# slitvinov/PINN_for_quantum_wavefunction_surfaces

Measured on NVIDIA B200. Metric: collocation points/sec per training step (fwd+lap+bwd), higher is better.
Workload: dtype f32

## Files before the change

pinn_for_quantum_wavefunction_surfaces_b200/csrc/pinn_device.cuh:

```cuda
#pragma once
#include "pinn_common.cuh"
#include "pinn_launch.h"

namespace pinn {

constexpr int ROWH = 64;
constexpr int ROWE = 32;
constexpr int EVAL_STASH = 2 * 32 * ROWH;
constexpr int ENET_STASH = 2 * 32 * ROWE;

__host__ __device__ constexpr int swz_tc(int row) { return ((((row & 3) << 1) | ((row >> 2) & 1)) << 2); }

__device__ __forceinline__ float rcp_approx(float x) {
  float r;
  asm("rcp.approx.ftz.f32 %0, %1;" : "=f"(r) : "f"(x));
  return r;
}
constexpr float NEG_LOG2E = -1.4426950408889634f;
__device__ __forceinline__ float ex2_approx(float x) {
  float e;
  asm("ex2.approx.ftz.f32 %0, %1;" : "=f"(e) : "f"(x));
  return e;
}

// ... 31 lines not shown
__device__ __forceinline__ float2 f2bc(float x) { return make_float2(x, x); }
__device__ __forceinline__ float2 f2neg(float2 a) { return make_float2(-a.x, -a.y); }
__device__ __forceinline__ float2 f2mul(float2 a, float2 b) { return __fmul2_rn(a, b); }
__device__ __forceinline__ float2 f2add(float2 a, float2 b) { return __fadd2_rn(a, b); }
__device__ __forceinline__ float2 f2fma(float2 a, float2 b, float2 c) { return __ffma2_rn(a, b, c); }

template <int ROW>
__device__ __forceinline__ float2 colsum2(const float* __restrict__ base, int col2, int half) {
  const float* b = base + half * 16 * ROW;
  float2 s0 = make_float2(0.0f, 0.0f), s1 = make_float2(0.0f, 0.0f);
#pragma unroll
  for (int p = 0; p < 16; p += 2) {
    s0 = __fadd2_rn(s0, *reinterpret_cast<const float2*>(b + p * ROW + (col2 ^ swz_tc(p))));
    s1 = __fadd2_rn(s1, *reinterpret_cast<const float2*>(b + (p + 1) * ROW + (col2 ^ swz_tc(p + 1))));
  }
  return __fadd2_rn(s0, s1);
}
template <int ROW>
__device__ __forceinline__ void colsum2_w(const float* __restrict__ base, int col2, int half, float wgt, float2& plain,
                                          float2& weighted) {
  const float* b = base + half * 16 * ROW;
  float2 s0 = make_float2(0.0f, 0.0f), s1 = s0, t0 = s0, t1 = s0;
  const int r0 = half * 16;
#pragma unroll
  for (int p = 0; p < 16; p += 2) {
    const float2 v0 = *reinterpret_cast<const float2*>(b + p * ROW + (col2 ^ swz_tc(p)));
    const float2 v1 = *reinterpret_cast<const float2*>(b + (p + 1) * ROW + (col2 ^ swz_tc(p + 1)));
    const float w0 = __shfl_sync(0xffffffffu, wgt, r0 + p), w1 = __shfl_sync(0xffffffffu, wgt, r0 + p + 1);
    s0 = __fadd2_rn(s0, v0); s1 = __fadd2_rn(s1, v1);
    t0 = __ffma2_rn(v0, make_float2(w0, w0), t0);
    t1 = __ffma2_rn(v1, make_float2(w1, w1), t1);
  }
  plain = __fadd2_rn(s0, s1);
  weighted = __fadd2_rn(t0, t1);
}

struct Geom {
  float f1, f2, ir1, ir2, al1, al2, al11, al12, al22;
  float R;
};

struct RawPt {
  float dx1, dx2, y, z, R;
};
__device__ __forceinline__ RawPt load_raw(const StepParams& p, long long i) {
  RawPt r;
  if (p.in_f64) {
    const double xd = ((const double*)p.x)[i], Rd = ((const double*)p.R)[i];
    r.dx1 = (float)(xd - Rd);
    r.dx2 = (float)(xd + Rd);
    r.y = (float)((const double*)p.y)[i];
    r.z = (float)((const double*)p.z)[i];
    r.R = (float)Rd;
  } else {
    const float xf = ((const float*)p.x)[i];
    r.R = ((const float*)p.R)[i];
    r.dx1 = xf - r.R;
    r.dx2 = xf + r.R;
    r.y = ((const float*)p.y)[i];
    r.z = ((const float*)p.z)[i];
  }
  return r;
}
__device__ __forceinline__ Geom geom_from_raw(const RawPt& r) {
  Geom g;
  const float yz = fmaf(r.y, r.y, r.z * r.z);
  const float q1 = fmaf(r.dx1, r.dx1, yz), q2 = fmaf(r.dx2, r.dx2, yz);
  g.ir1 = rsqrtf(q1);
  g.ir2 = rsqrtf(q2);
  const float r1 = q1 * g.ir1, r2 = q2 * g.ir2;
  g.f1 = __expf(-r1);
  g.f2 = __expf(-r2);
  const float c12 = fmaf(r.dx1, r.dx2, yz) * g.ir1 * g.ir2;
  g.al1 = g.f1 * fmaf(-2.0f, g.ir1, 1.0f);
  g.al2 = g.f2 * fmaf(-2.0f, g.ir2, 1.0f);
  g.al11 = g.f1 * g.f1;
  g.al22 = g.f2 * g.f2;
  g.al12 = 2.0f * g.f1 * g.f2 * c12;
  g.R = r.R;
  return g;
}
__device__ __forceinline__ Geom load_geom(const StepParams& p, long long i) { return geom_from_raw(load_raw(p, i)); }

__device__ __forceinline__ void build_weight_image(const float* __restrict__ th, Wts* __restrict__ out, int t, int nt) {
  for (int i = t; i < NH; i += nt) {
    const float a = th[O_W1 + 2 * i], b = th[O_W1 + 2 * i + 1];
    out->w0[i] = a; out->w1[i] = b; out->b1[i] = th[O_B1 + i];
    out->ww00[i] = a * a; out->ww01[i] = a * b; out->ww11[i] = b * b;
    out->b2[i] = th[O_B2 + i]; out->wo[i] = th[O_WO + i];
    out->w0s[i] = a * NEG_LOG2E; out->w1s[i] = b * NEG_LOG2E;
    out->b1s[i] = th[O_B1 + i] * NEG_LOG2E; out->b2s[i] = th[O_B2 + i] * NEG_LOG2E;
  }
  for (int i = t; i < NE; i += nt) {
    out->WE1[i] = th[O_WE1 + i]; out->bE1[i] = th[O_BE1 + i];
    out->bE2[i] = th[O_BE2 + i]; out->wE[i] = th[O_WE + i];
    out->WE1s[i] = th[O_WE1 + i] * NEG_LOG2E; out->bE1s[i] = th[O_BE1 + i] * NEG_LOG2E;
    out->bE2s[i] = th[O_BE2 + i] * NEG_LOG2E;
  }
  for (int i = t; i < 12; i += nt) {
    const bool in = i < NL;
    out->WgL[i] = in ? th[O_WGL + i] : 0.0f;
    out->bgL[i] = in ? th[O_BGL + i] : 0.0f;
    out->wg[i] = in ? th[O_WG + i] : 0.0f;
    out->WgLs[i] = in ? th[O_WGL + i] * NEG_LOG2E : 0.0f;
    out->bgLs[i] = in ? th[O_BGL + i] * NEG_LOG2E : 0.0f;
  }
  if (t == 0) { out->bo = th[O_BO]; out->bE = th[O_BE]; out->bg = th[O_BG]; out->pad0 = 0.0f; }
  auto put = [](float* hi, float* lo, int off, float v) {
    uint32_t h, l;
    split_tf32_rn(v, h, l);
    hi[off] = __uint_as_float(h);
    lo[off] = __uint_as_float(l);
  };
  for (int i = t; i < NH * NH; i += nt) {
    const int j = i / NH, k = i % NH;
    const float wjk = th[O_W2 + i];
    const float a = th[O_W1 + 2 * k], b = th[O_W1 + 2 * k + 1];
    put(out->BS[0], out->BS[1], umma_off(j, k, NH), wjk);
    put(out->BSP[0], out->BSP[1], umma_off(j, k, 2 * NH), wjk * a);
    put(out->BSP[0], out->BSP[1], umma_off(NH + j, k, 2 * NH), wjk * b);
    put(out->BSPP[0], out->BSPP[1], umma_off(j, k, 3 * NH), wjk * (a * a));
    put(out->BSPP[0], out->BSPP[1], umma_off(NH + j, k, 3 * NH), wjk * (a * b));
    put(out->BSPP[0], out->BSPP[1], umma_off(2 * NH + j, k, 3 * NH), wjk * (b * b));
    put(out->BWT[0], out->BWT[1], umma_off(k, j, NH), wjk);
  }
  for (int i = t; i < NE * NE; i += nt) {
    const int j = i / NE, k = i % NE;
    put(out->BE[0], out->BE[1], umma_off(j, k, NE), th[O_WE2 + i]);
    put(out->BET[0], out->BET[1], umma_off(k, j, NE), th[O_WE2 + i]);
  }
}

__device__ __forceinline__ void st_relaxed_sys_v2(unsigned int* p, unsigned int a, unsigned int b) {
  asm volatile("st.relaxed.sys.global.v2.u32 [%0], {%1, %2};" ::"l"(p), "r"(a), "r"(b) : "memory");
}
__device__ __forceinline__ uint2 ld_relaxed_sys_v2(const unsigned int* p) {
  uint2 v;
  asm volatile("ld.relaxed.sys.global.v2.u32 {%0, %1}, [%2];" : "=r"(v.x), "=r"(v.y) : "l"(p) : "memory");
  return v;
}
__device__ __forceinline__ double ld_acquire_gpu(const double* p) {
  double v;
  asm volatile("ld.acquire.gpu.global.f64 %0, [%1];" : "=d"(v) : "l"(p) : "memory");
  return v;
}
__device__ __forceinline__ void st_release_sys(unsigned long long* p, unsigned long long v) {
  asm volatile("st.release.sys.global.u64 [%0], %1;" ::"l"(p), "l"(v) : "memory");
}
__device__ __forceinline__ unsigned long long ld_acquire_sys(const unsigned long long* p) {
  unsigned long long v;
  asm volatile("ld.acquire.sys.global.u64 %0, [%1];" : "=l"(v) : "l"(p) : "memory");
  return v;
}

__device__ __forceinline__ float2 sigm2_pre(const float2 up) {
  const float2 d = __fadd2_rn(make_float2(ex2_approx(up.x), ex2_approx(up.y)), make_float2(1.0f, 1.0f));
  return make_float2(rcp_approx(d.x), rcp_approx(d.y));
}

__device__ __forceinline__ float2 one_minus_sigm2(const float2 e, const float2 s) {
  return make_float2(__saturatef(__fmul_rn(e.x, s.x)), __saturatef(__fmul_rn(e.y, s.y)));
}

__device__ __forceinline__ float2 sigm2_pre(const float2 up, float2& om) {
  const float2 e = make_float2(ex2_approx(up.x), ex2_approx(up.y));
  const float2 d = __fadd2_rn(e, make_float2(1.0f, 1.0f));
  const float2 s = make_float2(rcp_approx(d.x), rcp_approx(d.y));
  om = one_minus_sigm2(e, s);
  return s;
}

__device__ __forceinline__ float2 one_minus_sigm2_pre(const float2 up, const float2 s) {
  return one_minus_sigm2(make_float2(ex2_approx(up.x), ex2_approx(up.y)), s);
}

__device__ __forceinline__ float2 quad_form2(float al11, float al12, float al22, float2 v1, float2 v2) {
  return f2fma(f2mul(f2bc(al11), v1), v1, f2fma(f2mul(f2bc(al12), v1), v2, f2mul(f2mul(f2bc(al22), v2), v2)));
}

#define LD4(ptr) (*reinterpret_cast<const float4*>(ptr))
#define ST4(ptr, a, b, c, d) (*reinterpret_cast<float4*>(ptr) = make_float4(a, b, c, d))

}
```

pinn_for_quantum_wavefunction_surfaces_b200/csrc/pinn_step_tc.cu:

```cuda
#include <cstring>
#include <type_traits>

#include "pinn_tc.cuh"

#ifdef PINN_TIMELINE
__device__ long long g_timeline[16 * 32];
#define TL(i) do { if (blockIdx.x == 0 && c.tl_it == 3 && (threadIdx.x & 31) == 0) g_timeline[(threadIdx.x >> 5) * 32 + (i)] = clock64(); } while (0)
extern "C" int pinn_debug_timeline(long long* out) { return (int)cudaMemcpyFromSymbol(out, g_timeline, sizeof(g_timeline)); }
__device__ long long g_timeline_k[48];
__device__ long long g_timeline_cta[2 * 256];
extern "C" int pinn_debug_timeline_cta(long long* out) { return (int)cudaMemcpyFromSymbol(out, g_timeline_cta, sizeof(g_timeline_cta)); }
#define TLK(i) do { if (blockIdx.x == 0 && threadIdx.x == 0) g_timeline_k[(i)] = clock64(); \
                    if (threadIdx.x == 0 && ((i) == 0 || (i) == 41)) { unsigned long long t_; asm volatile("mov.u64 %0, %%globaltimer;" : "=l"(t_)); \
                      g_timeline_cta[blockIdx.x * 2 + ((i) == 41)] = (long long)t_; } } while (0)
extern "C" int pinn_debug_timeline_kernel(long long* out) { return (int)cudaMemcpyFromSymbol(out, g_timeline_k, sizeof(g_timeline_k)); }
#else
#define TL(i) do { } while (0)
#define TLK(i) do { } while (0)
#endif

namespace pinn {


template <int NEV>
__host__ __device__ constexpr int tc_group_stash_floats() { return NEV * EVAL_STASH + ENET_STASH; }
constexpr int GEO_BYTES = 2 * 128 * 12 * 4;
template <int NEV>
__host__ __device__ constexpr size_t tc_smem_bytes() {
  return sizeof(Wts) + 64  + sizeof(float2) * 4 * 2 * 3 * 32 + sizeof(float) * 4 * tc_group_stash_floats<NEV>() +
         COORD_STAGES * COORD_STAGE_BYTES + GEO_BYTES;
}

__device__ __forceinline__ void cp_async4(uint32_t dst, const void* src) {
  asm volatile("cp.async.ca.shared.global [%0], [%1], 4;" ::"r"(dst), "l"(src) : "memory");
}
__device__ __forceinline__ void cp_async8(uint32_t dst, const void* src) {
  asm volatile("cp.async.ca.shared.global [%0], [%1], 8;" ::"r"(dst), "l"(src) : "memory");
}
__device__ __forceinline__ void cp_async_commit() { asm volatile("cp.async.commit_group;" ::: "memory"); }
__device__ __forceinline__ void cp_async_wait_all() { asm volatile("cp.async.wait_group 0;" ::: "memory"); }

__device__ __forceinline__ void coord_stage_issue(const StepParams& p, unsigned char* buf, int slot, long long i) {
  const uint32_t b = smem_u32(buf);
  if (p.in_f64) {
    cp_async8(b + 0 * COORD_COL_BYTES + slot * 8, (const double*)p.x + i);
    cp_async8(b + 1 * COORD_COL_BYTES + slot * 8, (const double*)p.y + i);
    cp_async8(b + 2 * COORD_COL_BYTES + slot * 8, (const double*)p.z + i);
    cp_async8(b + 3 * COORD_COL_BYTES + slot * 8, (const double*)p.R + i);
  } else {
    cp_async4(b + 0 * COORD_COL_BYTES + slot * 4, (const float*)p.x + i);
    cp_async4(b + 1 * COORD_COL_BYTES + slot * 4, (const float*)p.y + i);
    cp_async4(b + 2 * COORD_COL_BYTES + slot * 4, (const float*)p.z + i);
    cp_async4(b + 3 * COORD_COL_BYTES + slot * 4, (const float*)p.R + i);
  }
  if (p.mask) cp_async4(b + 4 * COORD_COL_BYTES + slot * 4, (const void*)((uintptr_t)(p.mask + i) & ~(uintptr_t)3));
}
__device__ __forceinline__ void coord_stage_issue_bulk(const StepParams& p, unsigned char* buf, uint64_t* bar, long long st) {
  const uint32_t b = smem_u32(buf), mb = smem_u32(bar);
  const uint32_t colb = p.in_f64 ? 1024u : 512u;
  const uint32_t total = 4u * colb + (p.mask ? 128u : 0u);
  asm volatile("fence.proxy.async.shared::cta;" ::: "memory");
  asm volatile("mbarrier.arrive.expect_tx.shared::cta.b64 _, [%0], %1;" ::"r"(mb), "r"(total) : "memory");
  const char* src[4] = {(const char*)p.x, (const char*)p.y, (const char*)p.z, (const char*)p.R};
#pragma unroll
  for (int c = 0; c < 4; c++)
    asm volatile("cp.async.bulk.shared::cluster.global.mbarrier::complete_tx::bytes [%0], [%1], %2, [%3];" ::"r"(b + c * COORD_COL_BYTES),
                 "l"(src[c] + (size_t)st * colb), "r"(colb), "r"(mb)
                 : "memory");
  if (p.mask)
    asm volatile("cp.async.bulk.shared::cluster.global.mbarrier::complete_tx::bytes [%0], [%1], %2, [%3];" ::"r"(b + 4 * COORD_COL_BYTES),
                 "l"(p.mask + (size_t)st * 128), "r"(128u), "r"(mb)
                 : "memory");
}
__device__ __forceinline__ RawPt coord_stage_read(const StepParams& p, const unsigned char* buf, int slot) {
  RawPt r;
  if (p.in_f64) {
    const double xd = *(const double*)(buf + 0 * COORD_COL_BYTES + slot * 8), Rd = *(const double*)(buf + 3 * COORD_COL_BYTES + slot * 8);
    r.dx1 = (float)(xd - Rd);
    r.dx2 = (float)(xd + Rd);
    r.y = (float)*(const double*)(buf + 1 * COORD_COL_BYTES + slot * 8);
    r.z = (float)*(const double*)(buf + 2 * COORD_COL_BYTES + slot * 8);
    r.R = (float)Rd;
  } else {
    const float xf = *(const float*)(buf + 0 * COORD_COL_BYTES + slot * 4);
    r.R = *(const float*)(buf + 3 * COORD_COL_BYTES + slot * 4);
    r.dx1 = xf - r.R;
    r.dx2 = xf + r.R;
    r.y = *(const float*)(buf + 1 * COORD_COL_BYTES + slot * 4);
    r.z = *(const float*)(buf + 2 * COORD_COL_BYTES + slot * 4);
  }
  return r;
}

__device__ __forceinline__ void tc_role_sync(const TcCtx& c) {
  tc_wait_st();
  tc_fence_before();
  if (c.issuer) named_barrier(c.bar_id, 128);
  else asm volatile("bar.arrive %0, %1;" ::"r"(c.bar_id), "r"(128) : "memory");
}

template <bool STASH>
// ... 506 lines not shown
      ch[20 + i] = gs.x; ch[20 + i + 1] = gs.y;
    }
    ch[30] = gate_grads ? gbar : 0.0f;
    ch[31] = Ebar;
#pragma unroll
    for (int c4 = 0; c4 < 32; c4 += 4) ST4(&E1row[c4 ^ sx], ch[c4], ch[c4 + 1], ch[c4 + 2], ch[c4 + 3]);
  }
  __syncwarp();
  {
    float2 plain, weighted;
    colsum2_w<ROWE>(Vs, 2 * (lane & 15), lane >> 4, R, plain, weighted);
    acc2(acc.s2, weighted);
    acc2(acc.s3, plain);
  }
  acc2(acc.s4, colsum2<ROWE>(E1s, 2 * (lane & 15), lane >> 4));
  __syncwarp();
}

template <typename EntryOf>
__device__ __forceinline__ void fold_pair(float* __restrict__ myrow, float2 v, int lane, EntryOf entry_of) {
  v.x += __shfl_xor_sync(0xffffffffu, v.x, 16);
  v.y += __shfl_xor_sync(0xffffffffu, v.y, 16);
  if (lane < 16) {
    const int a = entry_of(2 * lane), b = entry_of(2 * lane + 1);
    if (a >= 0) myrow[a] = v.x;
    if (b >= 0) myrow[b] = v.y;
  }
}

constexpr int TC_REG_MLP = 184, TC_REG_ENET = 136;
static_assert(128 * TC_REG_ENET + 256 * TC_REG_MLP <= 384 * 168, "register rebalancing must fit the launch allocation");

struct TcParamsPlain {
  StepParams p;
  double w[4];
};
struct TcParamsInline {
  StepParams p;
  double w[4];
  alignas(16) float theta[NTHETA + 3];
};

template <int NEV, bool TRAIN, bool INLINE>
__global__ void __launch_bounds__((NEV + 1) * 128, 1)
pinn_step_tc_kernel(const __grid_constant__ typename std::conditional<INLINE, TcParamsInline, TcParamsPlain>::type q) {
  const StepParams& p = q.p;
  constexpr int G = 4;
  extern __shared__ __align__(128) unsigned char smem_raw[];
  Wts& w = *reinterpret_cast<Wts*>(smem_raw);
  uint64_t* mbars = reinterpret_cast<uint64_t*>(smem_raw + sizeof(Wts));
  uint32_t* tmem_slot = reinterpret_cast<uint32_t*>(smem_raw + sizeof(Wts) + 32);
  uint64_t* cfull = reinterpret_cast<uint64_t*>(smem_raw + sizeof(Wts) + 40);
  float2* mbox = reinterpret_cast<float2*>(smem_raw + sizeof(Wts) + 64);
  float* stash = reinterpret_cast<float*>(smem_raw + sizeof(Wts) + 64 + sizeof(float2) * G * 2 * 3 * 32);
  unsigned char* cstage = smem_raw + tc_smem_bytes<NEV>() - COORD_STAGES * COORD_STAGE_BYTES - GEO_BYTES;
  float4* geo = reinterpret_cast<float4*>(smem_raw + tc_smem_bytes<NEV>() - GEO_BYTES);

  const int tid = threadIdx.x, lane = tid & 31;
  const int warp = __shfl_sync(0xffffffffu, tid >> 5, 0);
  const int role = warp >> 2, grp = warp & 3;
  const bool is_mlp = role < NEV;
  const int sx = swz_tc(lane);
  TLK(0);
  uint32_t* clk0_slot = reinterpret_cast<uint32_t*>(smem_raw + sizeof(Wts) + 36);
  unsigned long long* ns0_slot = reinterpret_cast<unsigned long long*>(smem_raw + sizeof(Wts) + 56);
  if (blockIdx.x == 0 && tid == 0) {
    unsigned long long ns0;
    asm volatile("mov.u64 %0, %%globaltimer;" : "=l"(ns0));
    *ns0_slot = ns0;
    *clk0_slot = (uint32_t)clock();
  }

  if (warp == 0) {
    asm volatile("tcgen05.alloc.cta_group::1.sync.aligned.shared::cta.b32 [%0], 512;" ::"r"(smem_u32(tmem_slot)) : "memory");
    asm volatile("tcgen05.relinquish_alloc_permit.cta_group::1.sync.aligned;" ::: "memory");
  }
  if (tid == 32) {
#pragma unroll
    for (int i = 0; i < 4; i++) asm volatile("mbarrier.init.shared::cta.b64 [%0], 1;" ::"r"(smem_u32(&mbars[i])));
#pragma unroll
    for (int i = 0; i < COORD_STAGES; i++) asm volatile("mbarrier.init.shared::cta.b64 [%0], 1;" ::"r"(smem_u32(&cfull[i])));
    asm volatile("fence.mbarrier_init.release.cluster;" ::: "memory");
  }
  tc_fence_before();
  __syncthreads();
  tc_fence_after();
  pdl_wait();
  const int slot = grp * 32 + lane;
  const bool stager = !is_mlp && !p.grid.on;
  const bool cbulk = INLINE && TRAIN && !p.grid.on &&
                     ((((uintptr_t)p.x | (uintptr_t)p.y | (uintptr_t)p.z | (uintptr_t)p.R | (uintptr_t)p.mask) & 15u) == 0);
  auto tile_bulk = [&](long long st) { return INLINE && cbulk && (st * 128 + 128 <= p.n); };
  const bool bulk_issuer = stager && grp == 0 && lane == 0;
  if (stager && tile_bulk(blockIdx.x)) {
    if (bulk_issuer) coord_stage_issue_bulk(p, cstage, &cfull[0], blockIdx.x);
  } else if (stager) {
    const long long i0 = (long long)blockIdx.x * 128 + slot;
    coord_stage_issue(p, cstage, slot, i0 < p.n ? i0 : p.n - 1);
    cp_async_commit();
  }

  {
    float* th_s = stash;
    constexpr uint32_t TH_BULK = (NTHETA * 4 / 16) * 16;
    const bool bulk_ok = ((uintptr_t)p.theta & 15u) == 0;
    if constexpr (INLINE) {
      const float4* src = reinterpret_cast<const float4*>(q.theta);
      for (int j = warp; j < (NTHETA + 3) / 4; j += (NEV + 1) * 4) {
        const float4 v = src[j];
        const float val = lane == 0 ? v.x : lane == 1 ? v.y : lane == 2 ? v.z : v.w;
        if (lane < 4 && 4 * j + lane < NTHETA) th_s[4 * j + lane] = val;
      }
    } else if (p.theta_from_tensors) {
      for (int i = tid; i < NTHETA; i += blockDim.x) {
        int k, off;
        theta_locate(i, k, off);
        int j = i - off;
        if (p.tensors_in_out) j = in_out_index(k, j);
        th_s[i] = p.tensors_f64 ? (float)static_cast<const double*>(p.theta_tensors[k])[j]
                                : static_cast<const float*>(p.theta_tensors[k])[j];
      }
    } else if (bulk_ok) {
      if (tid == 32) {
        asm volatile("mbarrier.arrive.expect_tx.shared::cta.b64 _, [%0], %1;" ::"r"(smem_u32(&mbars[0])), "r"(TH_BULK) : "memory");
        asm volatile(
            "cp.async.bulk.shared::cluster.global.mbarrier::complete_tx::bytes [%0], [%1], %2, [%3];" ::"r"(smem_u32(th_s)),
            "l"(p.theta), "r"(TH_BULK), "r"(smem_u32(&mbars[0]))
            : "memory");
      }
      for (int i = TH_BULK / 4 + tid; i < NTHETA; i += blockDim.x) th_s[i] = p.theta[i];
      mbar_wait(smem_u32(&mbars[0]), 0);
    } else {
      for (int i = tid; i < NTHETA; i += blockDim.x) th_s[i] = p.theta[i];
    }
    __syncthreads();
    build_weight_image(th_s, &w, tid, blockDim.x);
    asm volatile("fence.proxy.async.shared::cta;" ::: "memory");
    __syncthreads();
  }

  auto run_role = [&](auto mlp_tag) {
    constexpr bool IS_MLP = decltype(mlp_tag)::value;
    TcCtx c;
    c.tbase = __shfl_sync(0xffffffffu, *tmem_slot, 0);
    c.tlane = c.tbase + ((uint32_t)(grp * 32) << 16);
    c.mbar = smem_u32(&mbars[1 + role]);
    c.phase = 0;
    c.bar_id = 5 + role;
    c.issuer = (grp == 0);
    c.wts_saddr = smem_u32(&w);
    const uint32_t cb = IS_MLP ? (uint32_t)role * TC_MLP_COLS : TC_E_BASE;

    float* gstash = stash + grp * tc_group_stash_floats<NEV>();
    float* Hs = gstash + (IS_MLP ? role * EVAL_STASH : NEV * EVAL_STASH);
    float* Gs = Hs + (IS_MLP ? 32 * ROWH : 32 * ROWE);
    float2* gbox = mbox + grp * (2 * 3 * 32);

    double wpde = 0.0, wbc1 = 0.0, wbc2 = 0.0;
    if (TRAIN) {
      if (INLINE || p.w_by_value) { wpde = q.w[0]; wbc1 = q.w[1]; wbc2 = q.w[2]; }
      else { wpde = p.weights[0]; wbc1 = p.weights[1]; wbc2 = p.weights[2]; }
    }
    const float w_pde = (float)wpde, w_bc1 = (float)wbc1, w_bc2 = (float)wbc2;
    const float sN = p.vc.sN, cL = p.vc.cL, cV = p.vc.cV, cE = p.vc.cE;

    TcAcc acc;
  #pragma unroll
    for (int a = 0; a < 2; a++)
  #pragma unroll
      for (int b = 0; b < 4; b++)
  #pragma unroll
        for (int cc = 0; cc < 4; cc++) acc.c[a][b][cc] = 0.0f;
    acc.s0 = acc.s1 = acc.s2 = acc.s3 = acc.s4 = make_float2(0.0f, 0.0f);

    double gs0 = 0.0, gs1 = 0.0, gs2 = 0.0, gs3 = 0.0, gs4 = 0.0;

    const long long nsuper = (p.n + 127) >> 7;
    int it = 0;
    if (stager) {
      cp_async_wait_all();
      if (tile_bulk(blockIdx.x)) mbar_wait(smem_u32(&cfull[0]), 0u);
    }
    __syncthreads();
    TLK(1);
    const bool enet_once = !TRAIN && p.grid.on && !p.grid.sph;
    if (enet_once) {
      if (!IS_MLP) {
        const float Rg = (float)p.grid.R;
        float gt;
        const float E = tc_enet_forward<false>(w, c, Rg, Hs + lane * ROWE, Gs + lane * ROWE, sx, gt);
        gbox[2 * 32 + lane] = make_float2(E, gt);
        gbox[3 * 32 + 2 * 32 + lane] = make_float2(E, gt);
        if (blockIdx.x == 0 && grp == 0 && lane == 0) p.grid.partials[8 * (size_t)gridDim.x] = (double)E;
      }
      named_barrier(1 + grp, (NEV + 1) * 32);
    }
    for (long long st = blockIdx.x; st < nsuper && !(enet_once && !IS_MLP); st += gridDim.x, ++it) {
      const long long pidx = st * 128 + slot;
      const bool valid = pidx < p.n;
      const long long pi = valid ? pidx : (p.n - 1);
      c.tl_it = it;
      TL(0);
      if (it < 38) TLK(2 + it);
      const unsigned char* cbuf = cstage + (it % COORD_STAGES) * COORD_STAGE_BYTES;
      const bool this_bulk = tile_bulk(st);
      Geom g;
      float cur_dx1, cur_dx2, mk_f = 0.0f;
      if (!TRAIN) {
        const RawPt raw = p.grid.on ? (p.grid.sph ? tc_sph_point(p.grid, pi) : tc_grid_point(p, pi)) : coord_stage_read(p, cbuf, slot);
        g = geom_from_raw(raw);
        cur_dx1 = raw.dx1; cur_dx2 = raw.dx2;
      } else {
        float4* gp = geo + ((it & 1) * 128 + slot) * 3;
        if (!IS_MLP) {
          const RawPt raw = p.grid.on ? tc_grid_point(p, pi) : coord_stage_read(p, cbuf, slot);
          g = geom_from_raw(raw);
          cur_dx1 = raw.dx1; cur_dx2 = raw.dx2;
          if (TRAIN && p.mask) {
            const unsigned mk = this_bulk ? (unsigned)cbuf[4 * COORD_COL_BYTES + slot]
                                          : *(const uint32_t*)(cbuf + 4 * COORD_COL_BYTES + slot * 4) >> (8u * (unsigned)((uintptr_t)(p.mask + pi) & 3u));
            mk_f = (float)(mk & 3u);
          }
          gp[0] = make_float4(g.f1, g.f2, g.ir1, g.ir2);
          gp[1] = make_float4(g.al1, g.al2, g.al11, g.al12);
          gp[2] = make_float4(g.al22, cur_dx1, cur_dx2, mk_f);
          asm volatile("bar.arrive %0, %1;" ::"r"(8 + grp), "r"((NEV + 1) * 32) : "memory");
        } else {
          named_barrier(8 + grp, (NEV + 1) * 32);
          const float4 q0 = gp[0], q1 = gp[1], q2 = gp[2];
          g.f1 = q0.x; g.f2 = q0.y; g.ir1 = q0.z; g.ir2 = q0.w;
          g.al1 = q1.x; g.al2 = q1.y; g.al11 = q1.z; g.al12 = q1.w;
          g.al22 = q2.x; cur_dx1 = q2.y; cur_dx2 = q2.z; mk_f = q2.w;
          g.R = 0.0f;
        }
      }
      if (stager) {
        const long long in = pidx + (long long)gridDim.x * 128;
        const long long stn = st + gridDim.x;
        if (stn < nsuper) {
          unsigned char* nbuf = cstage + ((it + 1) % COORD_STAGES) * COORD_STAGE_BYTES;
          if (tile_bulk(stn)) {
            if (bulk_issuer) coord_stage_issue_bulk(p, nbuf, &cfull[(it + 1) % COORD_STAGES], stn);
          } else {
            coord_stage_issue(p, nbuf, slot, in < p.n ? in : p.n - 1);
          }
        }
        cp_async_commit();
      }
      float2* box = gbox + (it & 1) * (3 * 32);

      const bool sw = (role == 1) && IS_MLP;
      const float a = sw ? g.f2 : g.f1, b = sw ? g.f1 : g.f2;
      const float al1 = sw ? g.al2 : g.al1, al2 = sw ? g.al1 : g.al2;
      const float al11 = sw ? g.al22 : g.al11, al22 = sw ? g.al11 : g.al22;
      const float al12 = g.al12;

      if (IS_MLP) {
        float Nv, Dv;
        tc_mlp_forward<TRAIN>(w, c, cb, a, b, al1, al2, al11, al12, al22, Hs + lane * ROWH, Gs + lane * ROWH, sx, Nv, Dv);
        box[role * 32 + lane] = make_float2(Nv, Dv);
      } else {
        float gt;
        const float E = tc_enet_forward<TRAIN>(w, c, g.R, Hs + lane * ROWE, Gs + lane * ROWE, sx, gt);
        box[2 * 32 + lane] = make_float2(E, gt);
      }
      TL(5);
      if (stager) {
        cp_async_wait_all();
        const long long stn = st + (long long)gridDim.x;
        if (stn < nsuper && tile_bulk(stn))
          mbar_wait(smem_u32(&cfull[(it + 1) % COORD_STAGES]), (uint32_t)((it + 1) / COORD_STAGES) & 1u);
      }
      named_barrier(1 + grp, enet_once ? NEV * 32 : (NEV + 1) * 32);
      TL(6);

      float2 m0 = box[lane];
      if (NEV == 2) { const float2 m1 = box[32 + lane]; m0.x += m1.x; m0.y += m1.y; }
      const float2 me = box[2 * 32 + lane];
      const float E = me.x, gate = me.y;
      const float N = fmaf(sN, m0.x, w.bo), DN = sN * m0.y;
      const float q = g.ir1 + g.ir2;
      const float fs = g.f1 + g.f2;
      const float psi = fmaf(gate, N, fs);
      const float lcao = fmaf(cL, fs, fmaf(cV - 2.0f * cL, fmaf(g.f1, g.ir1, g.f2 * g.ir2),
                                            cV * fmaf(g.f1, g.ir2, g.f2 * g.ir1)));
      const float inner = fmaf(cL, DN, cV * q * N);
      const float res = fmaf(gate, inner, fmaf(cE * E, psi, lcao));

      if (!TRAIN) {
        if (p.grid.sph) {
          if (role == 0) {
            const double wq = sph_weight(p.grid, pidx);
            const float hl = fmaf(-0.5f, fs, -fmaf(g.f1, g.ir2, g.f2 * g.ir1));
            const float hpsi = fmaf(gate, fmaf(-0.5f, DN, -q * N), hl);
            double v0 = wq * (double)(psi * hpsi), v1 = wq * (double)(psi * psi);
            double v2 = wq * (double)(fs * hl), v3 = wq * (double)(fs * fs);
  #pragma unroll
            for (int o = 16; o > 0; o >>= 1) {
              v0 += __shfl_xor_sync(0xffffffffu, v0, o); v1 += __shfl_xor_sync(0xffffffffu, v1, o);
              v2 += __shfl_xor_sync(0xffffffffu, v2, o); v3 += __shfl_xor_sync(0xffffffffu, v3, o);
            }
            if (lane == 0) {
              double* row = p.grid.partials + 8 * (size_t)(st * 4 + grp);
              row[0] = v0; row[1] = v1; row[2] = v2; row[3] = v3; row[5] = (double)E;
            }
          }
          continue;
        }
        if (p.grid.on) {
          if (valid && role == 0) {
            int ix, iy, iz;
            grid_ijk(p.grid, pi, ix, iy, iz);
            const double wq = p.grid.wx[ix] * p.grid.wy[iy] * p.grid.wz[iz];
            const float hl = fmaf(-0.5f, fs, -fmaf(g.f1, g.ir2, g.f2 * g.ir1));
            const float hpsi = fmaf(gate, fmaf(-0.5f, DN, -q * N), hl);
            const float vr = fmaf(-cur_dx1, g.ir1 * g.ir1 * g.ir1, cur_dx2 * g.ir2 * g.ir2 * g.ir2);
            gs0 += wq * (double)(psi * hpsi);
            gs1 += wq * (double)(psi * psi);
            gs2 += wq * (double)(fs * hl);
            gs3 += wq * (double)(fs * fs);
            gs4 += wq * (double)(vr * psi * psi);
          }
          continue;
        }
        if (valid) {
          if (role == 0) {
            if (p.psi) p.psi[pidx] = psi;
            if (p.lap) p.lap[pidx] = g.al1 + g.al2 + gate * DN;
            if (p.res) p.res[pidx] = res;
            if (p.hpsi)
              p.hpsi[pidx] = fmaf(gate, fmaf(-0.5f, DN, -q * N),
                                  fmaf(-0.5f, fs, -fmaf(g.f1, g.ir2, g.f2 * g.ir1)));
          } else if (!IS_MLP) {
            if (p.E_out) { if (p.E_f64) reinterpret_cast<double*>(p.E_out)[pidx] = (double)E; else p.E_out[pidx] = E; }
          }
        }
        continue;
      }

      float m1f, m2f;
      if (p.mask) {
        const unsigned mk = (unsigned)mk_f;
        m1f = (mk & 1u) ? 1.0f : 0.0f;
        m2f = (mk & 2u) ? 1.0f : 0.0f;
      } else {
        m1f = (g.ir1 * p.bcut <= 1.0f) ? 1.0f : 0.0f;
        m2f = (g.ir2 * p.bcut <= 1.0f) ? 1.0f : 0.0f;
      }
      const float vw = valid ? 1.0f : 0.0f;
      const float rbar = 2.0f * w_pde * res * vw;
      const float pbar = 2.0f * fmaf(w_bc1, m1f, w_bc2 * m2f) * psi * vw;
      if (IS_MLP) {
        const float lamN = fmaf(rbar, gate * fmaf(cV, q, cE * E), pbar * gate);
        const float lamD = rbar * cL * gate;
        float extra[8];
  #pragma unroll
        for (int i = 0; i < 8; i++) extra[i] = 0.0f;
        if (role == 0) {
          extra[0] = res * res * vw;
          extra[1] = psi * psi * m1f * vw;
          extra[2] = psi * psi * m2f * vw;
          extra[3] = E * vw;
          extra[4] = p.base_grads ? lamN : 0.0f;
          extra[5] = m1f * vw;
          extra[6] = m2f * vw;
        }
        if (p.base_grads) {
          tc_mlp_backward(w, c, cb, a, b, al1, al2, al11, al12, al22, sN * lamN, sN * lamD, Hs, Gs, lane, extra, acc);
        } else if (role == 0) {
          tc_mlp_extras_only(Hs, lane, extra, acc);
        }
      } else {
        if (valid && p.E_out) { if (p.E_f64) reinterpret_cast<double*>(p.E_out)[pidx] = (double)E; else p.E_out[pidx] = E; }
        const float gbar = fmaf(rbar, fmaf(cE * E, N, inner), pbar * N);
        const float Ebar = rbar * cE * psi;
        tc_enet_backward(w, c, g.R, Ebar, gbar, p.gate_grads != 0, Hs, Gs, lane, acc);
      }
      TL(15);
    }

    TLK(40);
    if (TRAIN && blockIdx.x == 0 && tid == 0) {
      unsigned long long ns1;
      asm volatile("mov.u64 %0, %%globaltimer;" : "=l"(ns1));
      double* tm = reinterpret_cast<double*>(mbox);
      tm[0] = (double)((uint32_t)clock() - *clk0_slot);
      tm[1] = (double)(ns1 - *ns0_slot);
    }
    pdl_launch_dependents();
    tc_fence_before();
    __syncthreads();
    if (warp == 0) {
      tc_fence_after();
      asm volatile("tcgen05.dealloc.cta_group::1.sync.aligned.b32 %0, 512;" ::"r"(c.tbase) : "memory");
    }
    if (!TRAIN) {
      if (p.grid.on && !p.grid.sph) {
        double* red = reinterpret_cast<double*>(stash);
        if (role == 0) {
  #pragma unroll
          for (int o = 16; o > 0; o >>= 1) {
            gs0 += __shfl_xor_sync(0xffffffffu, gs0, o); gs1 += __shfl_xor_sync(0xffffffffu, gs1, o);
            gs2 += __shfl_xor_sync(0xffffffffu, gs2, o); gs3 += __shfl_xor_sync(0xffffffffu, gs3, o);
            gs4 += __shfl_xor_sync(0xffffffffu, gs4, o);
          }
          if (lane == 0) { red[grp * 8 + 0] = gs0; red[grp * 8 + 1] = gs1; red[grp * 8 + 2] = gs2; red[grp * 8 + 3] = gs3; red[grp * 8 + 4] = gs4; }
        }
        __syncthreads();
        if (tid < 5) p.grid.partials[8 * (size_t)blockIdx.x + tid] = (red[tid] + red[8 + tid]) + (red[16 + tid] + red[24 + tid]);
      }
      return;
    }

    {
      float* myrow = stash + warp * NPART;
      const int gq = lane >> 2, tq = lane & 3;
      if (IS_MLP) {
  #pragma unroll
        for (int nt = 0; nt < 2; nt++) {
          const int j0 = gq, j1 = gq + 8, k0 = nt * 8 + 2 * tq, k1 = k0 + 1;
          myrow[O_W2 + j0 * NH + k0] = acc.c[0][nt][0] + acc.c[1][nt][0];
          myrow[O_W2 + j0 * NH + k1] = acc.c[0][nt][1] + acc.c[1][nt][1];
          myrow[O_W2 + j1 * NH + k0] = acc.c[0][nt][2] + acc.c[1][nt][2];
          myrow[O_W2 + j1 * NH + k1] = acc.c[0][nt][3] + acc.c[1][nt][3];
        }
        auto e0 = [](int i) { return i < 16 ? O_B2 + i : O_WO + i - 16; };
        auto e1 = [](int i) { return i < 16 ? O_W1 + 2 * i : O_W1 + 2 * (i - 16) + 1; };
        auto e2 = [role](int i) {
          if (i < 16) return (int)O_B1 + i;
          if (role != 0) return -1;
          const int e = i - 16;
          return e == 0 ? (int)S_RES2 : e == 1 ? (int)S_PSI1 : e == 2 ? (int)S_PSI2 : e == 3 ? (int)S_E
               : e == 4 ? (int)O_BO : e == 5 ? (int)S_CNT1 : e == 6 ? (int)S_CNT2 : -1;
        };
        fold_pair(myrow, acc.s0, lane, e0);
        fold_pair(myrow, acc.s1, lane, e1);
        fold_pair(myrow, acc.s2, lane, e2);
      } else {
  #pragma unroll
        for (int mt = 0; mt < 2; mt++)
  #pragma unroll
          for (int nt = 0; nt < 4; nt++) {
            const int j0 = mt * 16 + gq, j1 = j0 + 8, k0 = nt * 8 + 2 * tq, k1 = k0 + 1;
            myrow[O_WE2 + j0 * NE + k0] = acc.c[mt][nt][0];
            myrow[O_WE2 + j0 * NE + k1] = acc.c[mt][nt][1];
            myrow[O_WE2 + j1 * NE + k0] = acc.c[mt][nt][2];
            myrow[O_WE2 + j1 * NE + k1] = acc.c[mt][nt][3];
          }
        fold_pair(myrow, acc.s0, lane, [](int i) { return (int)O_WE + i; });
        fold_pair(myrow, acc.s1, lane, [](int i) { return (int)O_BE2 + i; });
        fold_pair(myrow, acc.s2, lane, [](int i) { return (int)O_WE1 + i; });
        fold_pair(myrow, acc.s3, lane, [](int i) { return (int)O_BE1 + i; });
        fold_pair(myrow, acc.s4, lane, [](int i) {
          return i < 10 ? (int)O_WGL + i : i < 20 ? (int)O_BGL + i - 10 : i < 30 ? (int)O_WG + i - 20 : i == 30 ? (int)O_BG : (int)O_BE;
        });
      }
    }
    __syncthreads();
    constexpr int nwarps = (NEV + 1) * G;
    double* row = p.partials + (size_t)blockIdx.x * NPART;
    for (int i = tid; i < NPART; i += blockDim.x) {
      int w0, w1;
      if (i < O_BO) { w0 = 0; w1 = NEV * G; }
      else if (i == O_BO || (i >= S_RES2 && i <= S_CNT2)) { w0 = 0; w1 = G; }
      else if (i < NTHETA) { w0 = NEV * G; w1 = nwarps; }
      else { w0 = 0; w1 = 0; }
      double sum = 0.0;
      for (int wv = w0; wv < w1; wv++) sum += (double)stash[wv * NPART + i];
      if (i >= NPART - 2 && blockIdx.x == 0) sum = reinterpret_cast<const double*>(mbox)[i - (NPART - 2)];
      row[i] = sum;
    }
    TLK(41);
  };
  constexpr bool REBALANCE = TRAIN && NEV == 2;
  if (is_mlp) {
    if constexpr (REBALANCE) asm volatile("setmaxnreg.inc.sync.aligned.u32 %0;" ::"n"(TC_REG_MLP));
    run_role(std::true_type{});
  } else {
    if constexpr (REBALANCE) asm volatile("setmaxnreg.dec.sync.aligned.u32 %0;" ::"n"(TC_REG_ENET));
    run_role(std::false_type{});
  }
}

template <int NEV, bool TRAIN, bool INLINE>
static cudaError_t launch_step_tc_t(const StepParams& p, int grid, cudaStream_t st) {
  auto kern = pinn_step_tc_kernel<NEV, TRAIN, INLINE>;
  constexpr size_t smem = tc_smem_bytes<NEV>();
  static bool configured[16] = {false};
  int dev = 0;
  cudaGetDevice(&dev);
  if (dev < 16 && !configured[dev]) {
    cudaError_t e = cudaFuncSetAttribute(kern, cudaFuncAttributeMaxDynamicSharedMemorySize, (int)smem);
    if (e != cudaSuccess) return e;
    configured[dev] = true;
  }
  if constexpr (INLINE) {
    TcParamsInline q;
    q.p = p;
    memcpy(q.theta, p.theta_inline, NTHETA * sizeof(float));
    q.theta[NTHETA] = q.theta[NTHETA + 1] = q.theta[NTHETA + 2] = 0.0f;
    q.w[0] = q.w[1] = q.w[2] = q.w[3] = 0.0;
    if (p.weights_inline) memcpy(q.w, p.weights_inline, 3 * sizeof(double));
    q.p.w_by_value = p.weights_inline != nullptr;
    return launch_pdl(kern, dim3(grid), dim3((NEV + 1) * 128), smem, st, q);
  } else {
    TcParamsPlain q;
    q.p = p;
    q.w[0] = q.w[1] = q.w[2] = q.w[3] = 0.0;
    if (p.weights_inline) memcpy(q.w, p.weights_inline, 3 * sizeof(double));
    q.p.w_by_value = p.weights_inline != nullptr;
    return launch_pdl(kern, dim3(grid), dim3((NEV + 1) * 128), smem, st, q);
  }
}

__global__ void grid_finish_kernel(const double* __restrict__ partials, int nrows, double* __restrict__ out) {
  const int t = threadIdx.x;
  if (t < 5) {
    double s = 0.0;
    for (int r = 0; r < nrows; r++) s += partials[8 * (size_t)r + t];
    out[t] = s;
  } else if (t == 5) {
    out[5] = partials[8 * (size_t)nrows];
  } else if (t < 8) {
    out[t] = 0.0;
  }
}
cudaError_t launch_grid_finish(const double* partials, int nrows, double* out, cudaStream_t st) {
  grid_finish_kernel<<<1, 32, 0, st>>>(partials, nrows, out);
  return cudaGetLastError();
}

__global__ void sph_finish_kernel(const double* __restrict__ partials, int nR, int rows_per_R, const double* __restrict__ Rs,
                                  double* __restrict__ out) {
  const long long t = (long long)blockIdx.x * blockDim.x + threadIdx.x;
  if (t >= 8ll * nR) return;
  const int k = (int)(t >> 3), slot = (int)(t & 7);
  const double* rows = partials + 8 * (size_t)k * rows_per_R;
  double v = 0.0;
  if (slot < 4) {
    for (int r = 0; r < rows_per_R; r++) v += rows[8 * (size_t)r + slot];
  } else if (slot == 5) {
    v = rows[5];
  }
  if (!(Rs[k] > 0.0)) v = __longlong_as_double(0x7ff8000000000000ll);
  out[t] = v;
}
cudaError_t launch_sph_finish(const double* partials, int nR, int rows_per_R, const double* Rs, double* out, cudaStream_t st) {
  const long long n = 8ll * nR;
  sph_finish_kernel<<<(unsigned)((n + 255) / 256), 256, 0, st>>>(partials, nR, rows_per_R, Rs, out);
  return cudaGetLastError();
}

cudaError_t launch_step_tc(int nev, bool train, const StepParams& p, int grid, cudaStream_t st) {
  if (train && p.theta_inline)
    return nev == 2 ? launch_step_tc_t<2, true, true>(p, grid, st) : launch_step_tc_t<1, true, true>(p, grid, st);
// ... 6 lines not shown
```

Measured before the change: 2.322 billion.

## Overlap weight-operand build and tail reduction using role-split named barriers

Splits weight image construction into layer and operand parts. In training, only the MLP warps build the tensor-core operand images, while the E-net warps proceed and wait on a named barrier only at the first iteration. The prologue barrier and the coordinate bulk issue move after the theta load. The epilogue replaces full-CTA syncs with per-role named barriers, so each role reduces its own partials from its stash rows and TMEM dealloc overlaps the reduction. This cuts block-wide synchronisation in the prologue and epilogue, at the cost of more intricate barrier counts that must match exactly. It also adds timeline probes.

Result: faster. 2.357 billion (median of 6 runs) (+1.5%).

```diff
diff --git a/pinn_for_quantum_wavefunction_surfaces_b200/csrc/pinn_device.cuh b/pinn_for_quantum_wavefunction_surfaces_b200/csrc/pinn_device.cuh
--- a/pinn_for_quantum_wavefunction_surfaces_b200/csrc/pinn_device.cuh
+++ b/pinn_for_quantum_wavefunction_surfaces_b200/csrc/pinn_device.cuh
@@ -137,7 +137,7 @@
 }
 __device__ __forceinline__ Geom load_geom(const StepParams& p, long long i) { return geom_from_raw(load_raw(p, i)); }
 
-__device__ __forceinline__ void build_weight_image(const float* __restrict__ th, Wts* __restrict__ out, int t, int nt) {
+__device__ __forceinline__ void build_weight_layers(const float* __restrict__ th, Wts* __restrict__ out, int t, int nt) {
   for (int i = t; i < NH; i += nt) {
     const float a = th[O_W1 + 2 * i], b = th[O_W1 + 2 * i + 1];
     out->w0[i] = a; out->w1[i] = b; out->b1[i] = th[O_B1 + i];
@@ -161,6 +161,8 @@
     out->bgLs[i] = in ? th[O_BGL + i] * NEG_LOG2E : 0.0f;
   }
   if (t == 0) { out->bo = th[O_BO]; out->bE = th[O_BE]; out->bg = th[O_BG]; out->pad0 = 0.0f; }
+}
+__device__ __forceinline__ void build_weight_operands(const float* __restrict__ th, Wts* __restrict__ out, int t, int nt) {
   auto put = [](float* hi, float* lo, int off, float v) {
     uint32_t h, l;
     split_tf32_rn(v, h, l);
diff --git a/pinn_for_quantum_wavefunction_surfaces_b200/csrc/pinn_step_tc.cu b/pinn_for_quantum_wavefunction_surfaces_b200/csrc/pinn_step_tc.cu
--- a/pinn_for_quantum_wavefunction_surfaces_b200/csrc/pinn_step_tc.cu
+++ b/pinn_for_quantum_wavefunction_surfaces_b200/csrc/pinn_step_tc.cu
@@ -7,16 +7,23 @@
 __device__ long long g_timeline[16 * 32];
 #define TL(i) do { if (blockIdx.x == 0 && c.tl_it == 3 && (threadIdx.x & 31) == 0) g_timeline[(threadIdx.x >> 5) * 32 + (i)] = clock64(); } while (0)
 extern "C" int pinn_debug_timeline(long long* out) { return (int)cudaMemcpyFromSymbol(out, g_timeline, sizeof(g_timeline)); }
-__device__ long long g_timeline_k[48];
+__device__ long long g_timeline_k[3 * 64];
+__device__ long long g_timeline_w[3 * 16 * 4];
 __device__ long long g_timeline_cta[2 * 256];
 extern "C" int pinn_debug_timeline_cta(long long* out) { return (int)cudaMemcpyFromSymbol(out, g_timeline_cta, sizeof(g_timeline_cta)); }
-#define TLK(i) do { if (blockIdx.x == 0 && threadIdx.x == 0) g_timeline_k[(i)] = clock64(); \
+__device__ __forceinline__ int tl_cta_slot() {
+  return blockIdx.x == 0 ? 0 : blockIdx.x == gridDim.x / 2 ? 1 : blockIdx.x == gridDim.x - 1 ? 2 : -1;
+}
+#define TLK(i) do { if (threadIdx.x == 0 && tl_cta_slot() >= 0) g_timeline_k[tl_cta_slot() * 64 + (i)] = clock64(); \
                     if (threadIdx.x == 0 && ((i) == 0 || (i) == 41)) { unsigned long long t_; asm volatile("mov.u64 %0, %%globaltimer;" : "=l"(t_)); \
                       g_timeline_cta[blockIdx.x * 2 + ((i) == 41)] = (long long)t_; } } while (0)
+#define TLW(i) do { if ((threadIdx.x & 31) == 0 && tl_cta_slot() >= 0) g_timeline_w[(tl_cta_slot() * 16 + (threadIdx.x >> 5)) * 4 + (i)] = clock64(); } while (0)
 extern "C" int pinn_debug_timeline_kernel(long long* out) { return (int)cudaMemcpyFromSymbol(out, g_timeline_k, sizeof(g_timeline_k)); }
+extern "C" int pinn_debug_timeline_warps(long long* out) { return (int)cudaMemcpyFromSymbol(out, g_timeline_w, sizeof(g_timeline_w)); }
 #else
 #define TL(i) do { } while (0)
 #define TLK(i) do { } while (0)
+#define TLW(i) do { } while (0)
 #endif
 
 namespace pinn {
@@ -689,26 +696,22 @@
     for (int i = 0; i < COORD_STAGES; i++) asm volatile("mbarrier.init.shared::cta.b64 [%0], 1;" ::"r"(smem_u32(&cfull[i])));
     asm volatile("fence.mbarrier_init.release.cluster;" ::: "memory");
   }
-  tc_fence_before();
-  __syncthreads();
-  tc_fence_after();
   pdl_wait();
+  TLK(43);
   const int slot = grp * 32 + lane;
   const bool stager = !is_mlp && !p.grid.on;
   const bool cbulk = INLINE && TRAIN && !p.grid.on &&
                      ((((uintptr_t)p.x | (uintptr_t)p.y | (uintptr_t)p.z | (uintptr_t)p.R | (uintptr_t)p.mask) & 15u) == 0);
   auto tile_bulk = [&](long long st) { return INLINE && cbulk && (st * 128 + 128 <= p.n); };
   const bool bulk_issuer = stager && grp == 0 && lane == 0;
-  if (stager && tile_bulk(blockIdx.x)) {
-    if (bulk_issuer) coord_stage_issue_bulk(p, cstage, &cfull[0], blockIdx.x);
-  } else if (stager) {
+  if (stager && !tile_bulk(blockIdx.x)) {
     const long long i0 = (long long)blockIdx.x * 128 + slot;
     coord_stage_issue(p, cstage, slot, i0 < p.n ? i0 : p.n - 1);
     cp_async_commit();
   }
 
+  float* th_s = stash;
   {
-    float* th_s = stash;
     constexpr uint32_t TH_BULK = (NTHETA * 4 / 16) * 16;
     const bool bulk_ok = ((uintptr_t)p.theta & 15u) == 0;
     if constexpr (INLINE) {
@@ -736,14 +739,27 @@
             : "memory");
       }
       for (int i = TH_BULK / 4 + tid; i < NTHETA; i += blockDim.x) th_s[i] = p.theta[i];
-      mbar_wait(smem_u32(&mbars[0]), 0);
     } else {
       for (int i = tid; i < NTHETA; i += blockDim.x) th_s[i] = p.theta[i];
     }
+    tc_fence_before();
     __syncthreads();
-    build_weight_image(th_s, &w, tid, blockDim.x);
+    tc_fence_after();
+    TLK(42);
+    if (stager && tile_bulk(blockIdx.x) && bulk_issuer) coord_stage_issue_bulk(p, cstage, &cfull[0], blockIdx.x);
+    if (!INLINE && !p.theta_from_tensors && bulk_ok) mbar_wait(smem_u32(&mbars[0]), 0);
+    TLK(44);
+    build_weight_layers(th_s, &w, tid, blockDim.x);
+    if (!TRAIN) build_weight_operands(th_s, &w, tid, blockDim.x);
+    if (!TRAIN) asm volatile("fence.proxy.async.shared::cta;" ::: "memory");
+    __syncthreads();
+    TLK(45);
+  }
+  if (TRAIN && is_mlp) {
+    build_weight_operands(th_s, &w, tid, NEV * 128);
     asm volatile("fence.proxy.async.shared::cta;" ::: "memory");
-    __syncthreads();
+    named_barrier(14, NEV * 128);
+    asm volatile("bar.arrive %0, %1;" ::"r"(15), "r"(NEV * 128 + 32) : "memory");
   }
 
   auto run_role = [&](auto mlp_tag) {
@@ -769,6 +785,7 @@
       else { wpde = p.weights[0]; wbc1 = p.weights[1]; wbc2 = p.weights[2]; }
     }
     const float w_pde = (float)wpde, w_bc1 = (float)wbc1, w_bc2 = (float)wbc2;
+
     const float sN = p.vc.sN, cL = p.vc.cL, cV = p.vc.cV, cE = p.vc.cE;
 
     TcAcc acc;
@@ -788,7 +805,7 @@
       cp_async_wait_all();
       if (tile_bulk(blockIdx.x)) mbar_wait(smem_u32(&cfull[0]), 0u);
     }
-    __syncthreads();
+    if (!TRAIN) __syncthreads();
     TLK(1);
     const bool enet_once = !TRAIN && p.grid.on && !p.grid.sph;
     if (enet_once) {
@@ -809,6 +826,7 @@
       c.tl_it = it;
       TL(0);
       if (it < 38) TLK(2 + it);
+      if (it == 0) TLW(0);
       const unsigned char* cbuf = cstage + (it % COORD_STAGES) * COORD_STAGE_BYTES;
       const bool this_bulk = tile_bulk(st);
       Geom g;
@@ -834,6 +852,7 @@
           asm volatile("bar.arrive %0, %1;" ::"r"(8 + grp), "r"((NEV + 1) * 32) : "memory");
         } else {
           named_barrier(8 + grp, (NEV + 1) * 32);
+          if (it == 0) TLK(46);
           const float4 q0 = gp[0], q1 = gp[1], q2 = gp[2];
           g.f1 = q0.x; g.f2 = q0.y; g.ir1 = q0.z; g.ir2 = q0.w;
           g.al1 = q1.x; g.al2 = q1.y; g.al11 = q1.z; g.al12 = q1.w;
@@ -867,6 +886,7 @@
         tc_mlp_forward<TRAIN>(w, c, cb, a, b, al1, al2, al11, al12, al22, Hs + lane * ROWH, Gs + lane * ROWH, sx, Nv, Dv);
         box[role * 32 + lane] = make_float2(Nv, Dv);
       } else {
+        if (TRAIN && c.issuer && it == 0) named_barrier(15, NEV * 128 + 32);
         float gt;
         const float E = tc_enet_forward<TRAIN>(w, c, g.R, Hs + lane * ROWE, Gs + lane * ROWE, sx, gt);
         box[2 * 32 + lane] = make_float2(E, gt);
@@ -987,6 +1007,8 @@
     }
 
     TLK(40);
+    TLW(1);
+    if (TRAIN && !IS_MLP && c.issuer && it == 0) named_barrier(15, NEV * 128 + 32);
     if (TRAIN && blockIdx.x == 0 && tid == 0) {
       unsigned long long ns1;
       asm volatile("mov.u64 %0, %%globaltimer;" : "=l"(ns1));
@@ -995,13 +1017,13 @@
       tm[1] = (double)(ns1 - *ns0_slot);
     }
     pdl_launch_dependents();
-    tc_fence_before();
-    __syncthreads();
-    if (warp == 0) {
-      tc_fence_after();
-      asm volatile("tcgen05.dealloc.cta_group::1.sync.aligned.b32 %0, 512;" ::"r"(c.tbase) : "memory");
-    }
-    if (!TRAIN) {
+    if constexpr (!TRAIN) {
+      tc_fence_before();
+      __syncthreads();
+      if (warp == 0) {
+        tc_fence_after();
+        asm volatile("tcgen05.dealloc.cta_group::1.sync.aligned.b32 %0, 512;" ::"r"(c.tbase) : "memory");
+      }
       if (p.grid.on && !p.grid.sph) {
         double* red = reinterpret_cast<double*>(stash);
         if (role == 0) {
@@ -1016,68 +1038,100 @@
         __syncthreads();
         if (tid < 5) p.grid.partials[8 * (size_t)blockIdx.x + tid] = (red[tid] + red[8 + tid]) + (red[16 + tid] + red[24 + tid]);
       }
-      return;
-    }
-
-    {
-      float* myrow = stash + warp * NPART;
-      const int gq = lane >> 2, tq = lane & 3;
+    } else {
+      TLK(47);
+      if (!IS_MLP) {
+        tc_fence_before();
+        asm volatile("bar.arrive %0, %1;" ::"r"(12), "r"((NEV + 1) * 128) : "memory");
+      }
+
+      {
+        float* myrow = IS_MLP ? Hs : Hs - O_WE1;
+        const int gq = lane >> 2, tq = lane & 3;
+        if (IS_MLP) {
+    #pragma unroll
+          for (int nt = 0; nt < 2; nt++) {
+            const int j0 = gq, j1 = gq + 8, k0 = nt * 8 + 2 * tq, k1 = k0 + 1;
+            myrow[O_W2 + j0 * NH + k0] = acc.c[0][nt][0] + acc.c[1][nt][0];
+            myrow[O_W2 + j0 * NH + k1] = acc.c[0][nt][1] + acc.c[1][nt][1];
+            myrow[O_W2 + j1 * NH + k0] = acc.c[0][nt][2] + acc.c[1][nt][2];
+            myrow[O_W2 + j1 * NH + k1] = acc.c[0][nt][3] + acc.c[1][nt][3];
+          }
+          auto e0 = [](int i) { return i < 16 ? O_B2 + i : O_WO + i - 16; };
+          auto e1 = [](int i) { return i < 16 ? O_W1 + 2 * i : O_W1 + 2 * (i - 16) + 1; };
+          auto e2 = [role](int i) {
+            if (i < 16) return (int)O_B1 + i;
+            if (role != 0) return -1;
+            const int e = i - 16;
+            return e == 0 ? (int)S_RES2 : e == 1 ? (int)S_PSI1 : e == 2 ? (int)S_PSI2 : e == 3 ? (int)S_E
+                 : e == 4 ? (int)O_BO : e == 5 ? (int)S_CNT1 : e == 6 ? (int)S_CNT2 : -1;
+          };
+          fold_pair(myrow, acc.s0, lane, e0);
+          fold_pair(myrow, acc.s1, lane, e1);
+          fold_pair(myrow, acc.s2, lane, e2);
+        } else {
+    #pragma unroll
+          for (int mt = 0; mt < 2; mt++)
+    #pragma unroll
+            for (int nt = 0; nt < 4; nt++) {
+              const int j0 = mt * 16 + gq, j1 = j0 + 8, k0 = nt * 8 + 2 * tq, k1 = k0 + 1;
+              myrow[O_WE2 + j0 * NE + k0] = acc.c[mt][nt][0];
+              myrow[O_WE2 + j0 * NE + k1] = acc.c[mt][nt][1];
+              myrow[O_WE2 + j1 * NE + k0] = acc.c[mt][nt][2];
+              myrow[O_WE2 + j1 * NE + k1] = acc.c[mt][nt][3];
+            }
+          fold_pair(myrow, acc.s0, lane, [](int i) { return (int)O_WE + i; });
+          fold_pair(myrow, acc.s1, lane, [](int i) { return (int)O_BE2 + i; });
+          fold_pair(myrow, acc.s2, lane, [](int i) { return (int)O_WE1 + i; });
+          fold_pair(myrow, acc.s3, lane, [](int i) { return (int)O_BE1 + i; });
+          fold_pair(myrow, acc.s4, lane, [](int i) {
+            return i < 10 ? (int)O_WGL + i : i < 20 ? (int)O_BGL + i - 10 : i < 30 ? (int)O_WG + i - 20 : i == 30 ? (int)O_BG : (int)O_BE;
+          });
+        }
+      }
+      TLK(48);
+      TLW(2);
+      constexpr int GS = tc_group_stash_floats<NEV>();
+      double* row = p.partials + (size_t)blockIdx.x * NPART;
+      uint32_t tix;
+      asm volatile("mov.u32 %0, %%tid.x;" : "=r"(tix));
       if (IS_MLP) {
+        tc_fence_before();
+        named_barrier(12, (NEV + 1) * 128);
+        TLK(49);
+        if (warp == 0) {
+          tc_fence_after();
+          asm volatile("tcgen05.dealloc.cta_group::1.sync.aligned.b32 %0, 512;" ::"r"(c.tbase) : "memory");
+        }
+        for (int j = (int)tix; j < O_BO + 1 + (NPART - NTHETA); j += NEV * 128) {
+          const int i = j <= O_BO ? j : j - (O_BO + 1) + NTHETA;
+          const int nw = i < O_BO ? NEV * G : (i == O_BO || (i >= S_RES2 && i <= S_CNT2)) ? G : 0;
+          float v[NEV * G];
   #pragma unroll
-        for (int nt = 0; nt < 2; nt++) {
-          const int j0 = gq, j1 = gq + 8, k0 = nt * 8 + 2 * tq, k1 = k0 + 1;
-          myrow[O_W2 + j0 * NH + k0] = acc.c[0][nt][0] + acc.c[1][nt][0];
-          myrow[O_W2 + j0 * NH + k1] = acc.c[0][nt][1] + acc.c[1][nt][1];
-          myrow[O_W2 + j1 * NH + k0] = acc.c[0][nt][2] + acc.c[1][nt][2];
-          myrow[O_W2 + j1 * NH + k1] = acc.c[0][nt][3] + acc.c[1][nt][3];
-        }
-        auto e0 = [](int i) { return i < 16 ? O_B2 + i : O_WO + i - 16; };
-        auto e1 = [](int i) { return i < 16 ? O_W1 + 2 * i : O_W1 + 2 * (i - 16) + 1; };
-        auto e2 = [role](int i) {
-          if (i < 16) return (int)O_B1 + i;
-          if (role != 0) return -1;
-          const int e = i - 16;
-          return e == 0 ? (int)S_RES2 : e == 1 ? (int)S_PSI1 : e == 2 ? (int)S_PSI2 : e == 3 ? (int)S_E
-               : e == 4 ? (int)O_BO : e == 5 ? (int)S_CNT1 : e == 6 ? (int)S_CNT2 : -1;
-        };
-        fold_pair(myrow, acc.s0, lane, e0);
-        fold_pair(myrow, acc.s1, lane, e1);
-        fold_pair(myrow, acc.s2, lane, e2);
+          for (int wv = 0; wv < NEV * G; wv++) v[wv] = stash[(wv & 3) * GS + (wv >> 2) * EVAL_STASH + i];
+          double sum = 0.0;
+  #pragma unroll
+          for (int wv = 0; wv < NEV * G; wv++)
+            if (wv < nw) sum += (double)v[wv];
+          if (i >= NPART - 2 && blockIdx.x == 0) sum = reinterpret_cast<const double*>(mbox)[i - (NPART - 2)];
+          row[i] = sum;
+        }
       } else {
+        named_barrier(13, 128);
+        for (int i = O_WE1 + ((int)tix - NEV * 128); i < NTHETA; i += 128) {
+          float v[G];
   #pragma unroll
-        for (int mt = 0; mt < 2; mt++)
+          for (int gv = 0; gv < G; gv++) v[gv] = stash[gv * GS + NEV * EVAL_STASH + (i - O_WE1)];
+          double sum = 0.0;
   #pragma unroll
-          for (int nt = 0; nt < 4; nt++) {
-            const int j0 = mt * 16 + gq, j1 = j0 + 8, k0 = nt * 8 + 2 * tq, k1 = k0 + 1;
-            myrow[O_WE2 + j0 * NE + k0] = acc.c[mt][nt][0];
-            myrow[O_WE2 + j0 * NE + k1] = acc.c[mt][nt][1];
-            myrow[O_WE2 + j1 * NE + k0] = acc.c[mt][nt][2];
-            myrow[O_WE2 + j1 * NE + k1] = acc.c[mt][nt][3];
-          }
-        fold_pair(myrow, acc.s0, lane, [](int i) { return (int)O_WE + i; });
-        fold_pair(myrow, acc.s1, lane, [](int i) { return (int)O_BE2 + i; });
-        fold_pair(myrow, acc.s2, lane, [](int i) { return (int)O_WE1 + i; });
-        fold_pair(myrow, acc.s3, lane, [](int i) { return (int)O_BE1 + i; });
-        fold_pair(myrow, acc.s4, lane, [](int i) {
-          return i < 10 ? (int)O_WGL + i : i < 20 ? (int)O_BGL + i - 10 : i < 30 ? (int)O_WG + i - 20 : i == 30 ? (int)O_BG : (int)O_BE;
-        });
-      }
-    }
-    __syncthreads();
-    constexpr int nwarps = (NEV + 1) * G;
-    double* row = p.partials + (size_t)blockIdx.x * NPART;
-    for (int i = tid; i < NPART; i += blockDim.x) {
-      int w0, w1;
-      if (i < O_BO) { w0 = 0; w1 = NEV * G; }
-      else if (i == O_BO || (i >= S_RES2 && i <= S_CNT2)) { w0 = 0; w1 = G; }
-      else if (i < NTHETA) { w0 = NEV * G; w1 = nwarps; }
-      else { w0 = 0; w1 = 0; }
-      double sum = 0.0;
-      for (int wv = w0; wv < w1; wv++) sum += (double)stash[wv * NPART + i];
-      if (i >= NPART - 2 && blockIdx.x == 0) sum = reinterpret_cast<const double*>(mbox)[i - (NPART - 2)];
-      row[i] = sum;
-    }
-    TLK(41);
+          for (int gv = 0; gv < G; gv++) sum += (double)v[gv];
+          row[i] = sum;
+        }
+      }
+      TLK(50);
+      TLW(3);
+      TLK(41);
+    }
   };
   constexpr bool REBALANCE = TRAIN && NEV == 2;
   if (is_mlp) {
```
